# zloyaloha/ray-tracing-practice

Hardware: AMD Instinct MI355X
Metric: Msamples/sec (pixels x spp / s), path-traced frame (higher is better)
Workload: dtype f32

## Files before the change

ray-tracing-practice_amd/csrc/rt_capi.hip:

```cpp
#include <hip/hip_runtime.h>

#include <cmath>
#include <cstdio>
#include <cstdlib>
#include <cstring>
#include <new>
#include <string>
#include <vector>

#include "../../include/rtp_amd.h"
#include "rt_accel.h"
#include "rt_build.h"
#include "rt_device_math.h"
#include "rt_kernel.hip.inc"
#include "rt_primary.hip.inc"
#include "rt_aov.hip.inc"
#include "rt_adaptive.hip.inc"
#include "rt_nee.hip.inc"
#include "rt_env.hip.inc"
#include "rt_light.hip.inc"

namespace {

thread_local std::string g_last_error;
// ... 187 lines not shown
    struct Feedback {
        uint32_t *host = nullptr; hipEvent_t start = nullptr, done = nullptr;
        bool pending = false, guarded = false, exploring = false;
        int passes = 0; uint64_t samples = 0, serial = 0;
    };
    Feedback feedback[kFeedbackSlots];
    int feedback_next = 0;
    double guarded_ns_per_sample = 0.0, exact_ns_per_sample = 0.0;
    bool explore_exact = false;
    uint64_t frame_serial = 0;
    uint32_t trip_test = 0;
    const uint32_t *last_traced_pixels = nullptr;
    int32_t last_spp = 0;
    float4 *leaf_boxes = nullptr, *plane_leaf_boxes = nullptr;
    uint32_t *flag_list = nullptr;
    uint32_t *resume_tag = nullptr; float4 *resume_state = nullptr;
    size_t flag_cap = 0;
    uint32_t *dirty = nullptr, *dirty_list = nullptr;
    size_t dirty_cap = 0;
    hipStream_t aux_stream = nullptr, list_stream = nullptr;
    hipEvent_t ev_fork = nullptr, ev_join = nullptr, ev_listed = nullptr;
    uint32_t *cand = nullptr;
    size_t cand_pixels = 0;
    struct CandKey { float view[12]; int32_t dims[9]; int repacks; hipStream_t stream; bool valid = false; } cand_key;
    int32_t num_internal = 0, num_spheres = 0, num_planes = 0, num_materials = 0, root = rtk::kDone, tree_depth = 0;
    CallClock clock[kNumClocks];
    std::vector<hipEvent_t> pass_events;
    int timed_passes = 0;
    rt_timing last{};
    int last_passes = 0;
    uint64_t last_samples = 0;
    bool timed = false;
    int num_cus = 0;
    uint64_t device_bytes = 0;
    float build_ms = 0.0f;
    bool absorbing_glass = false;
    std::vector<hipEvent_t> aov_events;
    float *adapt_mom = nullptr;
    uint32_t *adapt_list = nullptr, *adapt_work = nullptr, *adapt_counters = nullptr;
    size_t adapt_mom_pixels = 0, adapt_pixels = 0, adapt_work_cap = 0, adapt_counter_words = 0;
    bool nee_built = false;
    std::vector<int32_t> nee_index;
    std::vector<float> nee_cdf, nee_pmf;
    int32_t *nee_index_dev = nullptr;
    float *nee_cdf_dev = nullptr, *nee_pmf_dev = nullptr;
    std::vector<int32_t> emit_code;
    std::vector<float> emit_cdf, emit_pmf, emit_area;
    int32_t emit_spheres = 0, emit_planes = 0;
    int32_t *emit_code_dev = nullptr;
    float *emit_cdf_dev = nullptr, *emit_pmf_dev = nullptr, *emit_area_dev = nullptr;
};

namespace {

template <class T>
rt_status upload(const std::vector<T> &host, void **dev) {
// ... 124 lines not shown
        sc->repack_refused = true;
        return RT_OK;
    }
    HIP_TRY(hipStreamSynchronize(stream));
    float4 *nodes = nullptr, *hnodes = nullptr, *whnodes = nullptr, *leaf_boxes = nullptr, *plane_leaf_boxes = nullptr;
    rt_status st = RT_OK;
    if ((st = upload(pk.nodes, (void **)&nodes)) != RT_OK || (st = upload(pk.hnodes, (void **)&hnodes)) != RT_OK ||
        (st = upload(pk.whnodes, (void **)&whnodes)) != RT_OK ||
        (st = upload(pk.leaf_boxes, (void **)&leaf_boxes)) != RT_OK || (st = upload(pk.plane_leaf_boxes, (void **)&plane_leaf_boxes)) != RT_OK) {
        (void)hipFree(nodes); (void)hipFree(hnodes); (void)hipFree(whnodes); (void)hipFree(leaf_boxes); (void)hipFree(plane_leaf_boxes);
        return st;
    }
    (void)hipFree(sc->nodes); (void)hipFree(sc->hnodes); (void)hipFree(sc->whnodes);
    (void)hipFree(sc->leaf_boxes); (void)hipFree(sc->plane_leaf_boxes);
    sc->nodes = nodes; sc->hnodes = hnodes; sc->whnodes = whnodes; sc->leaf_boxes = leaf_boxes; sc->plane_leaf_boxes = plane_leaf_boxes;
    sc->num_wide = pk.num_wide; sc->wroot = pk.wroot; sc->wide_depth = pk.wide_depth;
    sc->num_internal = pk.num_internal;
    sc->num_top_pairs = pk.num_top_pairs;
    sc->root = pk.root;
    sc->tree_depth = pk.max_depth;
    sc->guard = pk.guard;
    sc->repacks++;
    return RT_OK;
}

}

__attribute__((visibility("hidden"))) void rt_internal_set_error(const std::string &msg) { g_last_error = msg; }

extern "C" {

const char *rt_get_last_error_string(void) { return g_last_error.c_str(); }

#if defined(RTP_PARITY_FLAGS) && !defined(__FAST_MATH__)
#define RTP_VERSION_PARITY "1"
#else
#define RTP_VERSION_PARITY "0"
#endif
#ifdef RTP_DEV_BUILD
#define RTP_VERSION_DEV "1"
#else
#define RTP_VERSION_DEV "0"
#endif
const char *rt_version_string(void) { return "rtp_amd 0.5 gfx950 parity=" RTP_VERSION_PARITY " dev=" RTP_VERSION_DEV; }

rt_status rt_set_device(int32_t device_ordinal) {
// ... 82 lines not shown
    if (cfg.guard_gamma_ulps < 0.0f || !(cfg.guard_gamma_ulps == cfg.guard_gamma_ulps)) return fail(RT_ERR_INVALID_ARG, "guard_gamma_ulps must be >= 0");
    rtaccel::Packed pk;
    const rtaccel::PackOptions popt = pack_options(cfg, desc);
    const bool device_build = cfg.tree_build == RT_BUILD_DEVICE_LBVH;
    std::string err = rtaccel::pack_scene(*desc, device_build ? rtaccel::TreeMode::GuardedLeaves : rtaccel::TreeMode::Guarded, pk, popt);
    if (!err.empty()) return fail(RT_ERR_INVALID_ARG, err);
    if (device_build && !pk.guard.ok) {
        err = rtaccel::pack_scene(*desc, rtaccel::TreeMode::Guarded, pk, popt);
        if (!err.empty()) return fail(RT_ERR_INVALID_ARG, err);
    }

    int n = 0;
    if (hipGetDeviceCount(&n) != hipSuccess || n <= 0) return fail(RT_ERR_NO_DEVICE, "no HIP device");
    rt_scene *sc = new (std::nothrow) rt_scene;
    if (!sc) return fail(RT_ERR_OUT_OF_MEMORY, "host allocation failed");
    sc->cfg = cfg;
    rt_status st = RT_OK;
    auto bail = [&](rt_status s) { rt_scene_destroy(sc); return s; };
    if (hipGetDevice(&sc->device) != hipSuccess) return bail(fail(RT_ERR_HIP, "hipGetDevice failed"));
    hipDeviceProp_t prop;
    if (hipGetDeviceProperties(&prop, sc->device) != hipSuccess) return bail(fail(RT_ERR_HIP, "hipGetDeviceProperties failed"));
    sc->num_cus = prop.multiProcessorCount;
    sc->device_bytes = (uint64_t)prop.totalGlobalMem;
    if (device_build && pk.guard.ok) {
        rtbuild::DeviceTree tree;
        const std::string berr = rtbuild::build_lbvh(pk.guard_leaf_boxes.data(), pk.guard_leaf_codes.data(), (int32_t)pk.guard_leaf_codes.size(), tree);
        if (!berr.empty()) return bail(fail(RT_ERR_HIP, "device BVH build: " + berr));
        sc->nodes = (float4 *)tree.nodes;
        sc->hnodes = (float4 *)tree.hnodes;
        pk.num_internal = tree.num_internal;
        pk.root = tree.root;
        pk.max_depth = tree.depth;
        pk.num_top_pairs = 0;
        sc->build_ms = tree.build_ms;
    } else {
        if ((st = upload(pk.nodes, (void **)&sc->nodes)) != RT_OK) return bail(st);
        if ((st = upload(pk.hnodes, (void **)&sc->hnodes)) != RT_OK) return bail(st);
        if ((st = upload(pk.whnodes, (void **)&sc->whnodes)) != RT_OK) return bail(st);
        sc->num_wide = pk.num_wide; sc->wroot = pk.wroot; sc->wide_depth = pk.wide_depth;
    }
    if ((st = upload(pk.tnodes, (void **)&sc->tnodes)) != RT_OK) return bail(st);
    sc->num_tnodes = pk.num_tnodes;
    if ((st = upload(pk.xnodes, (void **)&sc->xnodes)) != RT_OK) return bail(st);
    sc->num_top = pk.num_top;
    if ((st = upload(pk.spheres, (void **)&sc->spheres)) != RT_OK) return bail(st);
    if ((st = upload(pk.planes, (void **)&sc->planes)) != RT_OK) return bail(st);
// ... 15 lines not shown
        sc->device_built = device_build;
    }
    if (hipMalloc((void **)&sc->queue, kQueueWords * 4) != hipSuccess) return bail(fail(RT_ERR_OUT_OF_MEMORY, "hipMalloc(queue) failed"));
    if (sc->clock[kClockRender].make() != RT_OK) return bail(fail(RT_ERR_HIP, "hipEventCreate failed"));
    sc->num_internal = pk.num_internal;
    sc->num_top_pairs = pk.num_top_pairs;
    sc->num_spheres = (int32_t)pk.sphere_mat.size();
    sc->num_planes = (int32_t)(pk.planes.size() / 20);
    sc->num_materials = (int32_t)(pk.materials.size() / 12);
    sc->root = pk.root;
    sc->tree_depth = pk.max_depth;
    *out_scene = sc;
    return RT_OK;
}

rt_status rt_scene_destroy(rt_scene *sc) {
    if (!sc) return RT_OK;
    (void)hipFree(sc->tnodes);
    (void)hipFree(sc->xnodes);
    (void)hipFree(sc->nodes); (void)hipFree(sc->hnodes); (void)hipFree(sc->whnodes);
    (void)hipFree(sc->spheres); (void)hipFree(sc->planes); (void)hipFree(sc->materials);
    (void)hipFree(sc->sphere_mat); (void)hipFree(sc->tex_data); (void)hipFree(sc->tex_info); (void)hipFree(sc->queue); (void)hipFree(sc->slab);
    (void)hipFree(sc->leaf_boxes); (void)hipFree(sc->plane_leaf_boxes); (void)hipFree(sc->flag_list);
    (void)hipFree(sc->dirty); (void)hipFree(sc->dirty_list); (void)hipFree(sc->cand);
    (void)hipFree(sc->resume_tag); (void)hipFree(sc->resume_state);
    if (sc->aux_stream) (void)hipStreamDestroy(sc->aux_stream);
    if (sc->list_stream) (void)hipStreamDestroy(sc->list_stream);
    if (sc->ev_listed) (void)hipEventDestroy(sc->ev_listed);
    if (sc->ev_fork) (void)hipEventDestroy(sc->ev_fork);
    if (sc->ev_join) (void)hipEventDestroy(sc->ev_join);
    for (hipEvent_t e : sc->pass_events) (void)hipEventDestroy(e);
    for (hipEvent_t e : sc->aov_events) (void)hipEventDestroy(e);
    for (CallClock &c : sc->clock) c.destroy();
    (void)hipFree(sc->adapt_mom); (void)hipFree(sc->adapt_list); (void)hipFree(sc->adapt_work); (void)hipFree(sc->adapt_counters);
    (void)hipFree(sc->nee_index_dev); (void)hipFree(sc->nee_cdf_dev); (void)hipFree(sc->nee_pmf_dev);
    (void)hipFree(sc->emit_code_dev); (void)hipFree(sc->emit_cdf_dev); (void)hipFree(sc->emit_pmf_dev); (void)hipFree(sc->emit_area_dev);
    for (rt_scene::Feedback &f : sc->feedback) {
        if (f.done) { if (f.pending) (void)hipEventSynchronize(f.done); (void)hipEventDestroy(f.done); }
        if (f.start) (void)hipEventDestroy(f.start);
        if (f.host) (void)hipHostFree(f.host);
    }
    delete sc;
    return RT_OK;
}

const char *rt_scene_guard_reason(const rt_scene *sc) {
    if (!sc) return "null scene";
// ... 98 lines not shown
    if (plan.passes < 1) return fail(RT_ERR_UNSUPPORTED, "image too large for the work index arithmetic");
    if (plan.passes > kMaxPasses) return fail(RT_ERR_UNSUPPORTED, "more than 1024 passes (samples_per_pixel above 65536, or above 64512 at 2^24 pixels)");
    int pass_size = plan.pass_size;
    size_t need = (size_t)num_pixels * (size_t)slab_pitch_of(pass_size) * 3;
    if (sc->slab_floats < need) {
        HIP_TRY(hipStreamSynchronize(stream));
        (void)hipFree(sc->slab);
        sc->slab = nullptr;
        sc->slab_floats = 0;
        for (;;) {
            const hipError_t e = hipMalloc((void **)&sc->slab, need * sizeof(float));
            if (e == hipSuccess) break;
            (void)hipGetLastError();
            if (e != hipErrorOutOfMemory || pass_size <= 64) HIP_TRY(e);
            pass_size = pass_size / 2 < 64 ? 64 : pass_size / 2;
            plan = rtaccel::PassPlan::uniform(spp, pass_size);
            need = (size_t)num_pixels * (size_t)slab_pitch_of(pass_size) * 3;
        }
        sc->slab_floats = need;
    }
    return RT_OK;
}
rt_status reserve_view_lists(rt_scene *sc, uint32_t num_pixels, hipStream_t stream, bool &prim) {
    if (!prim || sc->cand_pixels >= (size_t)num_pixels) return RT_OK;
    HIP_TRY(hipStreamSynchronize(stream));
    (void)hipFree(sc->cand);
    sc->cand = nullptr;
    sc->cand_pixels = 0;
    sc->cand_key.valid = false;
    const size_t cand_words = (size_t)num_pixels * (rtk::kCandWords + 1) + 3 * (((size_t)num_pixels + rtk::kOrderBlock - 1) / rtk::kOrderBlock);
    if (hipMalloc((void **)&sc->cand, cand_words * sizeof(uint32_t)) == hipSuccess) {
        sc->cand_pixels = (size_t)num_pixels;
    } else {
        (void)hipGetLastError();
        sc->cand = nullptr;
        prim = false;
    }
    return RT_OK;
}
void bind_view_lists(const rt_scene *sc, rtk::KParams &P, uint32_t num_pixels, bool prim) {
    P.cand = prim ? sc->cand : nullptr;
    P.order = prim ? sc->cand + sc->cand_pixels * rtk::kCandWords : nullptr;
    P.traced_pixels = prim ? P.order + sc->cand_pixels + 2 * (((size_t)num_pixels + rtk::kOrderBlock - 1) / rtk::kOrderBlock) : nullptr;
}
rt_status make_view_lists(rt_scene *sc, const rt_camera_data *cam, const rtk::KParams &P, uint32_t num_pixels, hipStream_t stream) {
    rt_scene::CandKey key{};
    std::memcpy(key.view + 0, cam->origin.e, 12); std::memcpy(key.view + 3, cam->pixel00_loc.e, 12);
    std::memcpy(key.view + 6, cam->pixel_delta_u.e, 12); std::memcpy(key.view + 9, cam->pixel_delta_v.e, 12);
    const int32_t dims[9] = {P.width, P.height, P.local_rows, P.band_rows, P.num_parts, P.part, P.row_w, P.tile_x0, P.tile_y0};
    std::memcpy(key.dims, dims, sizeof(dims));
    key.repacks = sc->repacks; key.stream = stream; key.valid = true;
    const bool cand_cached = sc->cfg.reuse_view_lists >= 0 && sc->cand_key.valid && std::memcmp(key.view, sc->cand_key.view, sizeof(key.view)) == 0 &&
                             std::memcmp(key.dims, sc->cand_key.dims, sizeof(key.dims)) == 0 && key.repacks == sc->cand_key.repacks && key.stream == sc->cand_key.stream;
    if (cand_cached) return RT_OK;
    sc->cand_key.valid = false;
    const double coord_max = rtbeam::coord_bound(cam->origin.e, cam->pixel00_loc.e, cam->pixel_delta_u.e, cam->pixel_delta_v.e, cam->image_width, cam->image_height);
    hipLaunchKernelGGL(rtk::cand_kernel, dim3((num_pixels + 255u) / 256u), dim3(256), 0, stream, P, sc->cand, coord_max);
    HIP_TRY(hipGetLastError());
    uint32_t *order = sc->cand + sc->cand_pixels * rtk::kCandWords, *counts = order + sc->cand_pixels;
    const uint32_t order_blocks = (num_pixels + (uint32_t)rtk::kOrderBlock - 1u) / (uint32_t)rtk::kOrderBlock;
    hipLaunchKernelGGL(rtk::order_count_kernel, dim3(order_blocks), dim3(rtk::kOrderBlock), 0, stream, (const uint32_t *)sc->cand, num_pixels, order_blocks, counts);
    hipLaunchKernelGGL(rtk::order_scan_kernel, dim3(1), dim3(1024), 0, stream, counts, 3u * order_blocks);
    hipLaunchKernelGGL(rtk::order_scatter_kernel, dim3(order_blocks), dim3(rtk::kOrderBlock), 0, stream, (const uint32_t *)sc->cand, num_pixels, order_blocks,
                       (const uint32_t *)counts, order);
    HIP_TRY(hipGetLastError());
    sc->cand_key = key;
    return RT_OK;
}
void launch_primary(const rt_scene *sc, const rtk::KParams &P, uint32_t num_pixels, hipStream_t stream) {
    int pgrid = sc->num_cus * 8;
    const bool by_pixel = P.pass_count >= RTP_BY_PIXEL_MIN;
    const uint32_t units = by_pixel ? (num_pixels + 3u) / 4u : (P.total_work + 255u) / 256u;
    if ((uint32_t)pgrid > units) pgrid = (int)units;
    if (by_pixel) {
        if (P.num_planes > 0) hipLaunchKernelGGL(rtk::primary_pixel_kernel<true>, dim3(pgrid), dim3(256), 0, stream, P);
        else hipLaunchKernelGGL(rtk::primary_pixel_kernel<false>, dim3(pgrid), dim3(256), 0, stream, P);
    } else if (P.num_planes > 0) hipLaunchKernelGGL(rtk::primary_kernel<true>, dim3(pgrid), dim3(256), 0, stream, P);
    else hipLaunchKernelGGL(rtk::primary_kernel<false>, dim3(pgrid), dim3(256), 0, stream, P);
}

bool camera_within(const rt_camera_data *cam, const float c[3], double radius_sq) {
    const double dx = (double)cam->origin.e[0] - c[0], dy = (double)cam->origin.e[1] - c[1], dz = (double)cam->origin.e[2] - c[2];
    return dx * dx + dy * dy + dz * dz <= radius_sq;
}
bool camera_inside_margins(const rt_scene *sc, const rt_camera_data *cam) {
    return camera_within(cam, sc->guard.origin_center, (double)sc->guard.origin_radius * sc->guard.origin_radius) &&
           !(sc->guard.num_small > 0 && !camera_within(cam, sc->guard.center, (double)sc->guard.d0_sq * (1.0 - 1e-5)));
}
bool guarded_chosen(const rt_scene *sc, const rtk::KParams &P) {
    const rt_config &cfg = sc->cfg;
    return sc->guard.ok && cfg.traversal != RT_TRAVERSAL_EXACT && P.root >= 0 && guarded_wanted(cfg, (int64_t)P.num_spheres + P.num_planes) &&
           !(sc->guard_paused && !cfg.guard_keep);
}

rt_status choose_traversal(rt_scene *sc, const rt_camera_data *cam, const rt_shard *shard, const Tile *tile, hipStream_t stream, rtk::KParams &P,
                           bool &guarded, bool &exploring) {
    const rt_config &cfg = sc->cfg;
    guarded = guarded_chosen(sc, P);
    exploring = guarded && sc->explore_exact && cfg.traversal == RT_TRAVERSAL_AUTO && !cfg.guard_keep;
    if (exploring) guarded = false;
    if (!guarded) return RT_OK;
// ... 651 lines not shown
    bind_view_lists(sc, P, num_pixels, prim);
    CallClock &clock = sc->clock[kClockAov];
    if ((st = clock.make(1)) != RT_OK) return st;
    uint32_t *const walked = clock.words;
    const int timed = passes < kTimedPasses ? passes : kTimedPasses;
    if ((st = grow_events(sc->aov_events, 3 * (size_t)timed)) != RT_OK) return st;
    if ((st = clock.start(stream)) != RT_OK) return st;
    HIP_TRY(hipMemsetAsync(walked, 0, sizeof(uint32_t), stream));
    if (prim) {
        if ((st = make_view_lists(sc, cam, P, num_pixels, stream)) != RT_OK) return st;
    } else if (!lens) {
        sc->cand_key.valid = false;
    }
    for (int pass = 0; pass < passes; ++pass) {
        const bool timed_pass = pass < timed;
        if ((st = set_pass(P, plan, pass, num_pixels, sample_first)) != RT_OK) return st;
        if (timed_pass) HIP_TRY(hipEventRecord(sc->aov_events[3 * pass], stream));
        if (prim) {
            launch_primary(sc, P, num_pixels, stream);
            HIP_TRY(hipGetLastError());
        }
        if (timed_pass) HIP_TRY(hipEventRecord(sc->aov_events[3 * pass + 1], stream));
        const uint32_t units = prim ? (num_pixels + 3u) / 4u : (P.total_work + 255u) / 256u;
        const uint32_t rgrid = std::min<uint32_t>(units, (uint32_t)sc->num_cus * 8u);
        if (lens) hipLaunchKernelGGL(rtk::aov_resolve_lens_kernel, dim3(rgrid), dim3(256), 0, stream, P, *lens);
        else if (prim) hipLaunchKernelGGL(rtk::aov_resolve_kernel<false>, dim3(rgrid), dim3(256), 0, stream, P, walked);
        else hipLaunchKernelGGL(rtk::aov_resolve_kernel<true>, dim3(rgrid), dim3(256), 0, stream, P, walked);
        HIP_TRY(hipGetLastError());
        if (timed_pass) HIP_TRY(hipEventRecord(sc->aov_events[3 * pass + 2], stream));
        if (lens) hipLaunchKernelGGL(rtk::aov_accumulate_lens_kernel, acc_grid(num_pixels), dim3(64 * rtk::kAccWaves), 0, stream, P, *lens, out, pass == 0 ? 1 : 0, walked);
        else hipLaunchKernelGGL(rtk::aov_accumulate_kernel, acc_grid(num_pixels), dim3(64 * rtk::kAccWaves), 0, stream, P, out, pass == 0 ? 1 : 0, walked);
        HIP_TRY(hipGetLastError());
    }
    if ((st = clock.stop(stream)) != RT_OK) return st;
    rt_timing t{};
    t.primary_visibility = prim ? 1u : 0u;
    if (sync) {
        if ((st = clock.elapsed(t.kernel_ms)) != RT_OK) return st;
        float primary = 0.0f, rework = 0.0f, ms = 0.0f;
        for (int p = 0; p < timed; ++p) {
            HIP_TRY(hipEventElapsedTime(&ms, sc->aov_events[3 * p], sc->aov_events[3 * p + 1]));
            primary += ms;
            HIP_TRY(hipEventElapsedTime(&ms, sc->aov_events[3 * p + 1], sc->aov_events[3 * p + 2]));
            rework += ms;
        }
        primary *= untimed_scale(passes, timed);
        rework *= untimed_scale(passes, timed);
// ... 68 lines not shown
    if ((st = render_impl(sc, &base, shard, nullptr, d_fb_sum, hip_stream, 0, nullptr, 0, mom)) != RT_OK) return st;
    if (P.max_depth <= 0) {
        HIP_TRY(hipMemsetAsync(mom, 0, (size_t)num_pixels * 8, stream));
        HIP_TRY(hipMemsetD32Async((hipDeviceptr_t)d_spp, a.threshold == 0.0f ? a.min_spp + rounds * batch : a.min_spp, num_pixels, stream));
        if ((st = clock.stop(stream)) != RT_OK) return st;
        if (sync) HIP_TRY(hipStreamSynchronize(stream));
        return RT_OK;
    }
    if (sc->slab_floats < slab_need) return fail(RT_ERR_OUT_OF_MEMORY, "rt_render_adaptive: the sample slab shrank below a round's batch");

    if ((st = fill_params(sc, &base, shard, P)) != RT_OK) return st;
    const LaunchPlan plan = plan_launch(sc, &base, P, false);
    P.fb = d_fb_sum;
    bind_slab(sc, P, num_pixels, batch);
    set_exact_rewalk(P, sc->cfg, plan);
    P.cand = nullptr; P.order = nullptr; P.traced_pixels = nullptr;
    P.resume_tag = nullptr; P.resume_state = nullptr; P.abandon = nullptr; P.dirty = nullptr; P.dirty_list = nullptr;
    P.work_list = sc->adapt_work;
    P.work_cap = num_pixels * (uint32_t)batch;
    const void *exact = rewalk_kernel(plan);
    const int wgs = grid_for(sc, plan.exact, num_pixels, batch);
    const dim3 pix_grid((num_pixels + rtk::kAdaptBlock - 1) / rtk::kAdaptBlock), pix_block(rtk::kAdaptBlock);
    const uint64_t expand_items = (uint64_t)num_pixels * (uint64_t)batch;
    const uint32_t expand_grid = (uint32_t)std::min<uint64_t>((expand_items + rtk::kAdaptBlock - 1) / rtk::kAdaptBlock, (uint64_t)sc->num_cus * 8u);
    uint32_t *lists[2] = {sc->adapt_list, sc->adapt_list + num_pixels};
    uint32_t *const counters = sc->adapt_counters;
    HIP_TRY(hipMemsetAsync(counters, 0, (size_t)3 * (size_t)(rounds + 1) * sizeof(uint32_t), stream));
    int32_t n = a.min_spp;
    hipLaunchKernelGGL(rtk::adaptive_select_kernel<true>, pix_grid, pix_block, 0, stream, (const float *)mom, d_spp, num_pixels, (const uint32_t *)nullptr,
                       (const uint32_t *)nullptr, lists[0], counters, n, batch, a.max_spp, a.threshold);
    HIP_TRY(hipGetLastError());
    for (int32_t r = 1; r <= rounds; ++r) {
        const uint32_t *list = lists[(r - 1) & 1];
        const uint32_t *listed = counters + 3 * (r - 1);
        hipLaunchKernelGGL(rtk::adaptive_expand_kernel, dim3(expand_grid), pix_block, 0, stream, list, listed, (uint32_t)batch, sc->adapt_work,
                           counters + 3 * (r - 1) + 1);
        P.pass_first = n;
        P.pass_count = batch;
        P.total_work = num_pixels * (uint32_t)batch;
        if (!make_magic((uint32_t)batch, (uint64_t)P.total_work + 64, P.magic_count)) return fail(RT_ERR_UNSUPPORTED, "image too large for the work index arithmetic");
        P.work_count = counters + 3 * (r - 1) + 1;
        P.queue = counters + 3 * (r - 1) + 2;
        reservation(P.total_work, (uint64_t)wgs * (rtk::kBlock / rtk::kWave), P.full_chunk, P.full_taper);
        HIP_TRY(launch(exact, (uint32_t)rtk::kBlock, wgs, plan.exact.lds_bytes, stream, P));
        launch_accumulate(stream, P, Acc::onto_sums(list, listed));
        hipLaunchKernelGGL(rtk::moments_kernel<true>, pix_grid, pix_block, 0, stream, mom, (const float *)P.slab, num_pixels, P.slab_pitch, batch, 0, list, listed,
                           (const uint32_t *)nullptr, 0u, 0.0f, 0.0f, 0.0f);
// ... 1074 lines not shown
```

ray-tracing-practice_amd/csrc/rt_kernel.hip.inc:

```
#pragma once

namespace rtk {

using namespace rtd;

constexpr int kWave = 64;
constexpr int32_t kDone = INT32_MIN;
#ifndef RTP_BLOCK
#define RTP_BLOCK 768
#endif
#ifndef RTP_MIN_WAVES
#define RTP_MIN_WAVES 6
#endif
#ifndef RTP_UNROLL
#define RTP_UNROLL 4
#endif
#ifndef RTP_LDS_MAT_ROWS
#define RTP_LDS_MAT_ROWS 1
#endif
#ifndef RTP_UNROLL_WIDE
#define RTP_UNROLL_WIDE 3
#endif
#ifndef RTP_TRIPWIRE
#ifdef RTP_DEV_BUILD
// ... 120 lines not shown

__device__ __forceinline__ f3 inv_exact(const Lane &L) {
    f3 v = L.inv;
    if (__builtin_expect(!(fabsf(v.x) < 1e18f && fabsf(v.y) < 1e18f && fabsf(v.z) < 1e18f), 0)) v = mk(1.0f / L.d.x, 1.0f / L.d.y, 1.0f / L.d.z);
    return v;
}
template <bool kClamped = false>
__device__ __forceinline__ bool slab(const Lane &L0, float lox, float loy, float loz, float hix, float hiy, float hiz,
                                      float t_far, float &t_enter) {
    struct { f3 o, inv; } L = {L0.o, kClamped ? inv_exact(L0) : L0.inv};
    const bool sx = L.inv.x < 0, sy = L.inv.y < 0, sz = L.inv.z < 0;
    const float nx = sx ? hix : lox, fx = sx ? lox : hix;
    const float ny = sy ? hiy : loy, fy = sy ? loy : hiy;
    const float nz = sz ? hiz : loz, fz = sz ? loz : hiz;
    const float t1x = (nx - L.o.x) * L.inv.x, t2x = (fx - L.o.x) * L.inv.x;
    const float t1y = (ny - L.o.y) * L.inv.y, t2y = (fy - L.o.y) * L.inv.y;
    const float t1z = (nz - L.o.z) * L.inv.z, t2z = (fz - L.o.z) * L.inv.z;
    const float tmin = fmaxf(fmaxf(fmaxf(0.001f, t1x), t1y), t1z);
    const float tmax = fminf(fminf(fminf(t_far, t2x), t2y), t2z);
    t_enter = tmin;
    return tmax > tmin;
}

__device__ __forceinline__ bool slab_fused(f3 inv, f3 noi, float lox, float loy, float loz, float hix, float hiy, float hiz,
                                            float t_far, float &t_enter) {
    const float ax = __builtin_fmaf(lox, inv.x, noi.x), bx = __builtin_fmaf(hix, inv.x, noi.x);
    const float ay = __builtin_fmaf(loy, inv.y, noi.y), by = __builtin_fmaf(hiy, inv.y, noi.y);
    const float az = __builtin_fmaf(loz, inv.z, noi.z), bz = __builtin_fmaf(hiz, inv.z, noi.z);
    const float tmin = fmaxf(fmaxf(fminf(ax, bx), fminf(ay, by)), fmaxf(fminf(az, bz), 0.001f));
    const float tmax = fminf(fminf(fmaxf(ax, bx), fmaxf(ay, by)), fminf(fmaxf(az, bz), t_far));
    t_enter = tmin;
    return tmax > tmin;
}

constexpr int32_t kFlagBit = 1 << 30;
constexpr int32_t kEndBit = 1 << 25;
constexpr int32_t kFreshBit = 1 << 24;
constexpr int32_t kArmBit = 1 << 23;
constexpr int32_t kNoResumeBit = 1 << 22;
constexpr int32_t kMaxPrimDepth = 1 << 22;
constexpr int32_t kPrimMiss = -1;
constexpr int32_t kPrimFlag = -2;
constexpr int32_t kPrimWalk = -3;
#ifndef RTP_PRIM_ROUNDS
#define RTP_PRIM_ROUNDS 1
#endif
// ... 273 lines not shown
#endif

template <bool kGuard = false>
__device__ __forceinline__ void test_sphere(Lane &L, float4 s, int32_t prim) {
    const f3 oc = sub(L.o, mk(s.x, s.y, s.z));
    const float a = lensq(L.d);
    const float half_b = dot(oc, L.d);
    const float c = lensq(oc) - s.w * s.w;
    const float disc = half_b * half_b - a * c;
    if (disc < 0) return;
    const double sq = (double)sqrt_cr(disc);
    const double nb = (double)(-half_b);
    const double da = (double)a;
    float t;
    const bool ok = sphere_root(nb, sq, da, L.closest, t);
    if (ok) {
        if (kGuard && t == L.closest && L.hit >= 0) L.depth |= kFlagBit | RTP_WHY(1);
        L.closest = t;
        L.hit = prim;
    }
}

template <bool kGuard = false, bool kLazyFar = false>
__device__ __forceinline__ void test_sphere_ray(Lane &L, float4 s, int32_t prim, float a, double da, double y) {
    const f3 oc = sub(L.o, mk(s.x, s.y, s.z));
    const float half_b = dot(oc, L.d);
    const float c = lensq(oc) - s.w * s.w;
    const float disc = half_b * half_b - a * c;
    if (disc < 0) return;
    const double sq = (double)sqrt_cr(disc);
    const double nb = (double)(-half_b);
    float t;
    if (sphere_root_with<kLazyFar>(nb, sq, da, y, L.closest, t)) {
        if (kGuard && t == L.closest && L.hit >= 0) L.depth |= kFlagBit | RTP_WHY(1);
        L.closest = t;
        L.hit = prim;
    }
}

template <bool kGuard = false, class PlaneTab>
__device__ __forceinline__ void test_plane(Lane &L, PlaneTab planes, int32_t idx, int32_t prim) {
    const float4 P0 = planes[5 * idx + 0];
    const f3 n = mk(P0.x, P0.y, P0.z);
    const float denom = dot(n, L.d);
    if ((double)fabsf(denom) < 1e-8) return;
    const float t = (P0.w - dot(n, L.o)) / denom;
    if (!((0.001f <= t) && (t <= L.closest))) return;
    const float4 P1 = planes[5 * idx + 1];
    const float4 P2 = planes[5 * idx + 2];
    const float4 P3 = planes[5 * idx + 3];
    const float4 P4 = planes[5 * idx + 4];
    const f3 ph = sub(add(L.o, scale(t, L.d)), mk(P4.x, P4.y, P4.z));
    const f3 w = mk(P1.x, P1.y, P1.z);
    const float alpha = dot(w, cross(ph, mk(P3.x, P3.y, P3.z)));
    const float beta = dot(w, cross(mk(P2.x, P2.y, P2.z), ph));
    const int32_t type = as_int(P1.w);
    bool inside = true;
    if (type == RT_PLANE_QUAD) {
        inside = (0.0f <= alpha) && (alpha <= 1.0f) && (0.0f <= beta) && (beta <= 1.0f);
    } else if (type == RT_PLANE_ELLIPSE) {
// ... 869 lines not shown
```

ray-tracing-practice_amd/csrc/rt_primary.hip.inc:

```
#pragma once
#include "rt_beam.h"

namespace rtk {

constexpr int kCandWords = 16;
constexpr uint32_t kCandNone = 0xffffffffu;

__global__ void __launch_bounds__(256) cand_kernel(const KParams P, uint32_t *cand, double coord_max) {
    const uint32_t q = blockIdx.x * 256u + threadIdx.x;
    if (q >= P.num_pixels) return;
    const uint32_t pjl = q / (uint32_t)P.row_w;
    const int32_t pi = (int32_t)(q - pjl * (uint32_t)P.row_w) + P.tile_x0;
    int32_t pj = (int32_t)pjl + P.tile_y0;
    if (P.num_parts != 1) {
        const uint32_t band = pjl / (uint32_t)P.band_rows;
        pj = (int32_t)((band * (uint32_t)P.num_parts + (uint32_t)P.part) * (uint32_t)P.band_rows + (pjl - band * (uint32_t)P.band_rows));
    }
    const rtbeam::Beam beam = rtbeam::make_beam(P.origin, P.p00, P.du, P.dv, pi, pj, coord_max);
    uint32_t codes[kCandWords - 1];
    const float *tab = reinterpret_cast<const float *>(P.nodes);
    int n = rtbeam::beam_candidates(beam, [tab](int32_t k) { return tab + (size_t)k * 16; }, P.root, (double)P.g_dynk, codes, kCandWords - 1);
    n = rtbeam::beam_front_candidates(beam, P.num_front, P.front_code, P.front_box, (double)P.g_dynk, codes, n, kCandWords - 1);
    uint32_t *out = cand + (size_t)q * kCandWords;
    out[0] = n < 0 ? kCandNone : (uint32_t)n;
// ... 1 lines not shown
}

#ifndef RTP_ORDER_SPLIT
#define RTP_ORDER_SPLIT 1
#endif
constexpr int kOrderBlock = 256;
__device__ __forceinline__ uint32_t pixel_class(uint32_t n) { return n == 0u ? 2u : ((RTP_ORDER_SPLIT && n == 1u) ? 1u : 0u); }
__global__ void __launch_bounds__(kOrderBlock) order_count_kernel(const uint32_t *cand, uint32_t num_pixels, uint32_t num_blocks, uint32_t *counts) {
    __shared__ uint32_t part[3][kOrderBlock / 64];
    const uint32_t q = blockIdx.x * (uint32_t)kOrderBlock + threadIdx.x;
    const uint32_t cls = q < num_pixels ? pixel_class(cand[(size_t)q * kCandWords]) : 3u;
    const int wave = threadIdx.x >> 6;
    for (uint32_t c = 0; c < 3; ++c) {
        const uint32_t n = (uint32_t)__popcll(__ballot(cls == c));
        if ((threadIdx.x & 63) == 0) part[c][wave] = n;
    }
    __syncthreads();
    if (threadIdx.x < 3) {
        uint32_t n = 0;
        for (int w = 0; w < kOrderBlock / 64; ++w) n += part[threadIdx.x][w];
        counts[threadIdx.x * num_blocks + blockIdx.x] = n;
    }
}
__global__ void __launch_bounds__(1024) order_scan_kernel(uint32_t *counts, uint32_t n) {
    __shared__ uint32_t sums[1024];
    const uint32_t per = (n + 1023u) / 1024u;
    const uint32_t lo = threadIdx.x * per, hi = lo + per < n ? lo + per : n;
    uint32_t s = 0;
    for (uint32_t k = lo; k < hi; ++k) s += counts[k];
    sums[threadIdx.x] = s;
    __syncthreads();
    for (uint32_t d = 1; d < 1024u; d <<= 1) {
        const uint32_t v = threadIdx.x >= d ? sums[threadIdx.x - d] : 0u;
        __syncthreads();
        sums[threadIdx.x] += v;
        __syncthreads();
    }
    uint32_t run = sums[threadIdx.x] - s;
    for (uint32_t k = lo; k < hi; ++k) { const uint32_t c = counts[k]; counts[k] = run; run += c; }
}
__global__ void __launch_bounds__(kOrderBlock) order_scatter_kernel(const uint32_t *cand, uint32_t num_pixels, uint32_t num_blocks, const uint32_t *offsets,
                                                                    uint32_t *order) {
    __shared__ uint32_t part[3][kOrderBlock / 64];
    const uint32_t q = blockIdx.x * (uint32_t)kOrderBlock + threadIdx.x;
    const uint32_t cls = q < num_pixels ? pixel_class(cand[(size_t)q * kCandWords]) : 3u;
    const int wave = threadIdx.x >> 6;
    uint32_t rank = 0;
    for (uint32_t c = 0; c < 3; ++c) {
// ... 3 lines not shown
    }
    __syncthreads();
    if (cls < 3u) {
        for (int w = 0; w < wave; ++w) rank += part[cls][w];
        order[offsets[cls * num_blocks + blockIdx.x] + rank] = q;
    }
}

typedef __attribute__((address_space(4))) const uint32_t k_u32;
typedef float kf4 __attribute__((ext_vector_type(4)));
typedef __attribute__((address_space(4))) const kf4 k_f4;

struct RayConst { float a; double da, y; };
__device__ __forceinline__ RayConst ray_const(const Lane &L) {
    RayConst r;
    r.a = lensq(L.d);
    r.da = (double)r.a;
    r.y = sphere_root_rcp(r.da);
    return r;
}

typedef uint32_t ku4 __attribute__((ext_vector_type(4)));
typedef __attribute__((address_space(4))) const ku4 k_u4;
template <int C, bool kPlanes>
__device__ __forceinline__ void cand_step(Lane &L, const KParams &P, const RayConst &rc, k_u4 *list4, uint32_t n, k_f4 *sph, ku4 grp, float4 &hs) {
    if constexpr (C < kCandWords - 1) {
        if ((uint32_t)C >= n) return;
        if constexpr ((C + 1) % 4 == 0) grp = list4[(C + 1) / 4];
        const uint32_t code = grp[(C + 1) % 4];
        if (kPlanes && (code & 1u)) {
            test_plane<true>(L, P.planes, (int32_t)(code >> 1), (int32_t)code);
        } else {
            const kf4 sp = sph[code >> 1];
            test_sphere_ray<true, true>(L, make_float4(sp.x, sp.y, sp.z, sp.w), (int32_t)code, rc.a, rc.da, rc.y);
            const bool took = L.hit == (int32_t)code;
            hs = make_float4(took ? sp.x : hs.x, took ? sp.y : hs.y, took ? sp.z : hs.z, took ? sp.w : hs.w);
        }
        cand_step<C + 1, kPlanes>(L, P, rc, list4, n, sph, grp, hs);
    }
}
template <bool kPlanes>
__device__ __forceinline__ int32_t test_uniform_list(Lane &L, const KParams &P, uint32_t q0, float4 &hs) {
    k_u4 *list4 = (k_u4 *)(uintptr_t)(P.cand + (size_t)q0 * kCandWords);
    const ku4 first = list4[0];
    const uint32_t n = first.x;
    if (n == kCandNone) return kPrimWalk;
    const RayConst rc = ray_const(L);
    cand_step<0, kPlanes>(L, P, rc, list4, n, (k_f4 *)(uintptr_t)P.spheres, first, hs);
    return L.hit >= 0 ? L.hit : kPrimMiss;
}
template <bool kPlanes>
__device__ __forceinline__ int32_t test_lane_list(Lane &L, const KParams &P, uint32_t q, float4 &hs) {
    const uint32_t *list = P.cand + (size_t)q * kCandWords;
    const uint32_t n = list[0];
    if (n == kCandNone) return kPrimWalk;
    const RayConst rc = ray_const(L);
    for (uint32_t c = 0; c < n; ++c) {
        const uint32_t code = list[1 + c];
        const int32_t idx = (int32_t)(code >> 1);
        if (kPlanes && (code & 1u)) test_plane<true>(L, P.planes, idx, (int32_t)code);
        else {
            const float4 sp = P.spheres[idx];
            test_sphere_ray<true, true>(L, sp, (int32_t)code, rc.a, rc.da, rc.y);
            if (L.hit == (int32_t)code) hs = sp;
        }
    }
    return L.hit >= 0 ? L.hit : kPrimMiss;
}
template <bool kPlanes>
__device__ __forceinline__ void finish_primary(Lane &L, const KParams &P, int32_t code_out, uint32_t seed1, float4 hs, float *rec) {
    if (P.leaf_boxes == nullptr) {
        float enter;
        const bool in = slab(L, hs.x - hs.w, hs.y - hs.w, hs.z - hs.w, hs.x + hs.w, hs.y + hs.w, hs.z + hs.w, 1e30f, enter);
        const bool sphere_hit = code_out >= 0 && (!kPlanes || !(code_out & 1));
        if (sphere_hit && !(in && L.closest > enter)) L.depth |= kFlagBit;
        if (kPlanes && code_out >= 0 && (code_out & 1) && !guard_final_check<false>(L, P, P.spheres)) L.depth |= kFlagBit;
    } else if (code_out >= 0 && !guard_final_check<false>(L, P, P.spheres)) {
        L.depth |= kFlagBit;
    }
    if (L.depth & kFlagBit) code_out = kPrimFlag;
    rec[0] = L.closest;
    rec[1] = __int_as_float(code_out);
    rec[2] = __uint_as_float(seed1);
}

template <bool kPlanes>
__global__ void __launch_bounds__(256) primary_kernel(const KParams P) {
    const uint32_t lane = threadIdx.x & 63u;
    const uint32_t wave = (blockIdx.x * 256u + threadIdx.x) >> 6, num_waves = gridDim.x * 4u;
    const uint32_t batches = (P.total_work + 63u) >> 6;
    for (uint32_t b = wave; b < batches; b += num_waves) {
        const uint32_t w = b * 64u + lane;
        if (w >= P.total_work) continue;
        int32_t pi, pj;
        uint32_t k, record;
        map_work<false>(P, w, pi, pj, k, 0u, nullptr, nullptr, &record);
        const uint32_t q = P.pass_count == 64 ? (w >> 6) : div_magic(w, P.magic_count);
        if (P.cand[(size_t)q * kCandWords] == 0u) continue;
        Lane L;
        f3 ray_o, ray_d;
        const uint32_t seed1 = sample_seed1(wang_hash((uint32_t)pi * (uint32_t)P.width + (uint32_t)pj), P.pass_first + (int32_t)k);
        camera_ray<false>(L, P, pi, pj, seed1, ray_o, ray_d);
        begin_ray(L, ray_o, ray_d, 0);
        const uint32_t q0 = __builtin_amdgcn_readfirstlane(q);
        float4 hs = make_float4(0.0f, 0.0f, 0.0f, 0.0f);
        const int32_t code_out = __ballot(q != q0) == 0ull ? test_uniform_list<kPlanes>(L, P, q0, hs) : test_lane_list<kPlanes>(L, P, q, hs);
        finish_primary<kPlanes>(L, P, code_out, seed1, hs, P.slab + (size_t)record * 3);
    }
}

template <bool kPlanes>
__global__ void __launch_bounds__(256) primary_pixel_kernel(const KParams P) {
    const uint32_t lane = threadIdx.x & 63u;
    const uint32_t wave = __builtin_amdgcn_readfirstlane((blockIdx.x * 256u + threadIdx.x) >> 6), num_waves = gridDim.x * 4u;
    for (uint32_t q = wave; q < P.num_pixels; q += num_waves) {
        const uint32_t pjl = div_magic(q, P.magic_width);
        const int32_t pi = (int32_t)(q - pjl * (uint32_t)P.row_w) + P.tile_x0;
        int32_t pj = (int32_t)pjl + P.tile_y0;
        if (P.num_parts != 1) {
            const uint32_t band = div_magic(pjl, P.magic_band);
            pj = (int32_t)((band * (uint32_t)P.num_parts + (uint32_t)P.part) * (uint32_t)P.band_rows + (pjl - band * (uint32_t)P.band_rows));
        }
        float *row = P.slab + (size_t)q * P.slab_pitch * 3;
        if (*(k_u32 *)(uintptr_t)(P.cand + (size_t)q * kCandWords) == 0u) continue;
        const uint32_t base_seed = wang_hash((uint32_t)pi * (uint32_t)P.width + (uint32_t)pj);
        for (uint32_t k = lane; k < (uint32_t)P.pass_count; k += 64u) {
            Lane L;
            f3 ray_o, ray_d;
            const uint32_t seed1 = sample_seed1(base_seed, P.pass_first + (int32_t)k);
            camera_ray<false>(L, P, pi, pj, seed1, ray_o, ray_d);
            begin_ray(L, ray_o, ray_d, 0);
            float4 hs = make_float4(0.0f, 0.0f, 0.0f, 0.0f);
            const int32_t code_out = test_uniform_list<kPlanes>(L, P, q, hs);
            finish_primary<kPlanes>(L, P, code_out, seed1, hs, row + (size_t)k * 3);
        }
    }
}

}
```

Measured before the change: 12020.

## Precompute per-sphere camera-relative rows and size grids from occupancy

Adds a per-scene buffer of camera-relative sphere data (origin offset, c term, and box bounds), filled inside the order scan kernel, so primary rays test spheres and their slab boxes without recomputing origin subtraction and radius terms per sample. It adds a fast path for single-candidate pixels. Launch grids for the primary, AOV resolve and adaptive expand kernels are now sized from a measured occupancy query instead of a fixed 8 workgroups per CU. The trade-off is extra memory traffic of three float4 per sphere and possible slight differences in rounding from relative box bounds.

```diff
diff --git a/ray-tracing-practice_amd/csrc/rt_capi.hip b/ray-tracing-practice_amd/csrc/rt_capi.hip
--- a/ray-tracing-practice_amd/csrc/rt_capi.hip
+++ b/ray-tracing-practice_amd/csrc/rt_capi.hip
@@ -233,6 +233,7 @@
     hipEvent_t ev_fork = nullptr, ev_join = nullptr, ev_listed = nullptr;
     uint32_t *cand = nullptr;
     size_t cand_pixels = 0;
+    float4 *view_rows = nullptr;
     struct CandKey { float view[12]; int32_t dims[9]; int repacks; hipStream_t stream; bool valid = false; } cand_key;
     int32_t num_internal = 0, num_spheres = 0, num_planes = 0, num_materials = 0, root = rtk::kDone, tree_depth = 0;
     CallClock clock[kNumClocks];
@@ -243,6 +244,7 @@
     uint64_t last_samples = 0;
     bool timed = false;
     int num_cus = 0;
+    struct Residency { int primary_pixel[2] = {0, 0}, primary[2] = {0, 0}, aov_resolve[2] = {0, 0}, aov_resolve_lens = 0, adapt_expand = 0; } resident;
     uint64_t device_bytes = 0;
     float build_ms = 0.0f;
     bool absorbing_glass = false;
@@ -413,6 +415,34 @@
     sc->guard = pk.guard;
     sc->repacks++;
     return RT_OK;
+}
+
+#ifndef RTP_GRID_WGS_PER_CU
+#define RTP_GRID_WGS_PER_CU 0
+#endif
+rt_status resident_wgs(const void *kernel, int threads, int &out) {
+    int n = 0;
+    HIP_TRY(hipOccupancyMaxActiveBlocksPerMultiprocessor(&n, kernel, threads, 0));
+    if (n < 1) return fail(RT_ERR_HIP, "the occupancy query admits no workgroup of a kernel");
+    const int most = 2048 / threads;
+    out = RTP_GRID_WGS_PER_CU > 0 ? RTP_GRID_WGS_PER_CU : (n < most ? n : most);
+    return RT_OK;
+}
+rt_status measure_residency(rt_scene *sc) {
+    rt_scene::Residency &r = sc->resident;
+    rt_status st;
+    if ((st = resident_wgs(reinterpret_cast<const void *>(&rtk::primary_pixel_kernel<false>), 256, r.primary_pixel[0])) != RT_OK) return st;
+    if ((st = resident_wgs(reinterpret_cast<const void *>(&rtk::primary_pixel_kernel<true>), 256, r.primary_pixel[1])) != RT_OK) return st;
+    if ((st = resident_wgs(reinterpret_cast<const void *>(&rtk::primary_kernel<false>), 256, r.primary[0])) != RT_OK) return st;
+    if ((st = resident_wgs(reinterpret_cast<const void *>(&rtk::primary_kernel<true>), 256, r.primary[1])) != RT_OK) return st;
+    if ((st = resident_wgs(reinterpret_cast<const void *>(&rtk::aov_resolve_kernel<false>), 256, r.aov_resolve[0])) != RT_OK) return st;
+    if ((st = resident_wgs(reinterpret_cast<const void *>(&rtk::aov_resolve_kernel<true>), 256, r.aov_resolve[1])) != RT_OK) return st;
+    if ((st = resident_wgs(reinterpret_cast<const void *>(&rtk::aov_resolve_lens_kernel), 256, r.aov_resolve_lens)) != RT_OK) return st;
+    return resident_wgs(reinterpret_cast<const void *>(&rtk::adaptive_expand_kernel), rtk::kAdaptBlock, r.adapt_expand);
+}
+uint32_t resident_grid(const rt_scene *sc, int wgs_per_cu, uint64_t units) {
+    const uint64_t grid = (uint64_t)sc->num_cus * (uint64_t)wgs_per_cu;
+    return (uint32_t)(units < grid ? units : grid);
 }
 
 }
@@ -541,6 +571,7 @@
     if (hipGetDeviceProperties(&prop, sc->device) != hipSuccess) return bail(fail(RT_ERR_HIP, "hipGetDeviceProperties failed"));
     sc->num_cus = prop.multiProcessorCount;
     sc->device_bytes = (uint64_t)prop.totalGlobalMem;
+    if ((st = measure_residency(sc)) != RT_OK) return bail(st);
     if (device_build && pk.guard.ok) {
         rtbuild::DeviceTree tree;
         const std::string berr = rtbuild::build_lbvh(pk.guard_leaf_boxes.data(), pk.guard_leaf_codes.data(), (int32_t)pk.guard_leaf_codes.size(), tree);
@@ -602,7 +633,7 @@
     (void)hipFree(sc->spheres); (void)hipFree(sc->planes); (void)hipFree(sc->materials);
     (void)hipFree(sc->sphere_mat); (void)hipFree(sc->tex_data); (void)hipFree(sc->tex_info); (void)hipFree(sc->queue); (void)hipFree(sc->slab);
     (void)hipFree(sc->leaf_boxes); (void)hipFree(sc->plane_leaf_boxes); (void)hipFree(sc->flag_list);
-    (void)hipFree(sc->dirty); (void)hipFree(sc->dirty_list); (void)hipFree(sc->cand);
+    (void)hipFree(sc->dirty); (void)hipFree(sc->dirty_list); (void)hipFree(sc->cand); (void)hipFree(sc->view_rows);
     (void)hipFree(sc->resume_tag); (void)hipFree(sc->resume_state);
     if (sc->aux_stream) (void)hipStreamDestroy(sc->aux_stream);
     if (sc->list_stream) (void)hipStreamDestroy(sc->list_stream);
@@ -747,7 +778,15 @@
     return RT_OK;
 }
 rt_status reserve_view_lists(rt_scene *sc, uint32_t num_pixels, hipStream_t stream, bool &prim) {
-    if (!prim || sc->cand_pixels >= (size_t)num_pixels) return RT_OK;
+    if (!prim) return RT_OK;
+    if (sc->view_rows == nullptr && sc->num_spheres > 0 &&
+        hipMalloc((void **)&sc->view_rows, (size_t)sc->num_spheres * rtk::kViewRows * sizeof(float4)) != hipSuccess) {
+        (void)hipGetLastError();
+        sc->view_rows = nullptr;
+        prim = false;
+        return RT_OK;
+    }
+    if (sc->cand_pixels >= (size_t)num_pixels) return RT_OK;
     HIP_TRY(hipStreamSynchronize(stream));
     (void)hipFree(sc->cand);
     sc->cand = nullptr;
@@ -785,7 +824,8 @@
     uint32_t *order = sc->cand + sc->cand_pixels * rtk::kCandWords, *counts = order + sc->cand_pixels;
     const uint32_t order_blocks = (num_pixels + (uint32_t)rtk::kOrderBlock - 1u) / (uint32_t)rtk::kOrderBlock;
     hipLaunchKernelGGL(rtk::order_count_kernel, dim3(order_blocks), dim3(rtk::kOrderBlock), 0, stream, (const uint32_t *)sc->cand, num_pixels, order_blocks, counts);
-    hipLaunchKernelGGL(rtk::order_scan_kernel, dim3(1), dim3(1024), 0, stream, counts, 3u * order_blocks);
+    hipLaunchKernelGGL(rtk::order_scan_kernel, dim3(1), dim3(1024), 0, stream, counts, 3u * order_blocks, (const float4 *)P.spheres, (uint32_t)P.num_spheres, P.origin[0],
+                       P.origin[1], P.origin[2], sc->view_rows);
     hipLaunchKernelGGL(rtk::order_scatter_kernel, dim3(order_blocks), dim3(rtk::kOrderBlock), 0, stream, (const uint32_t *)sc->cand, num_pixels, order_blocks,
                        (const uint32_t *)counts, order);
     HIP_TRY(hipGetLastError());
@@ -793,15 +833,16 @@
     return RT_OK;
 }
 void launch_primary(const rt_scene *sc, const rtk::KParams &P, uint32_t num_pixels, hipStream_t stream) {
-    int pgrid = sc->num_cus * 8;
     const bool by_pixel = P.pass_count >= RTP_BY_PIXEL_MIN;
     const uint32_t units = by_pixel ? (num_pixels + 3u) / 4u : (P.total_work + 255u) / 256u;
-    if ((uint32_t)pgrid > units) pgrid = (int)units;
+    const int planes = P.num_planes > 0 ? 1 : 0;
+    const float4 *rows = sc->view_rows;
+    const uint32_t pgrid = resident_grid(sc, by_pixel ? sc->resident.primary_pixel[planes] : sc->resident.primary[planes], units);
     if (by_pixel) {
-        if (P.num_planes > 0) hipLaunchKernelGGL(rtk::primary_pixel_kernel<true>, dim3(pgrid), dim3(256), 0, stream, P);
-        else hipLaunchKernelGGL(rtk::primary_pixel_kernel<false>, dim3(pgrid), dim3(256), 0, stream, P);
-    } else if (P.num_planes > 0) hipLaunchKernelGGL(rtk::primary_kernel<true>, dim3(pgrid), dim3(256), 0, stream, P);
-    else hipLaunchKernelGGL(rtk::primary_kernel<false>, dim3(pgrid), dim3(256), 0, stream, P);
+        if (planes) hipLaunchKernelGGL(rtk::primary_pixel_kernel<true>, dim3(pgrid), dim3(256), 0, stream, P, rows);
+        else hipLaunchKernelGGL(rtk::primary_pixel_kernel<false>, dim3(pgrid), dim3(256), 0, stream, P, rows);
+    } else if (planes) hipLaunchKernelGGL(rtk::primary_kernel<true>, dim3(pgrid), dim3(256), 0, stream, P, rows);
+    else hipLaunchKernelGGL(rtk::primary_kernel<false>, dim3(pgrid), dim3(256), 0, stream, P, rows);
 }
 
 bool camera_within(const rt_camera_data *cam, const float c[3], double radius_sq) {
@@ -1499,7 +1540,7 @@
         }
         if (timed_pass) HIP_TRY(hipEventRecord(sc->aov_events[3 * pass + 1], stream));
         const uint32_t units = prim ? (num_pixels + 3u) / 4u : (P.total_work + 255u) / 256u;
-        const uint32_t rgrid = std::min<uint32_t>(units, (uint32_t)sc->num_cus * 8u);
+        const uint32_t rgrid = resident_grid(sc, lens ? sc->resident.aov_resolve_lens : sc->resident.aov_resolve[prim ? 0 : 1], units);
         if (lens) hipLaunchKernelGGL(rtk::aov_resolve_lens_kernel, dim3(rgrid), dim3(256), 0, stream, P, *lens);
         else if (prim) hipLaunchKernelGGL(rtk::aov_resolve_kernel<false>, dim3(rgrid), dim3(256), 0, stream, P, walked);
         else hipLaunchKernelGGL(rtk::aov_resolve_kernel<true>, dim3(rgrid), dim3(256), 0, stream, P, walked);
@@ -1614,7 +1655,7 @@
     const int wgs = grid_for(sc, plan.exact, num_pixels, batch);
     const dim3 pix_grid((num_pixels + rtk::kAdaptBlock - 1) / rtk::kAdaptBlock), pix_block(rtk::kAdaptBlock);
     const uint64_t expand_items = (uint64_t)num_pixels * (uint64_t)batch;
-    const uint32_t expand_grid = (uint32_t)std::min<uint64_t>((expand_items + rtk::kAdaptBlock - 1) / rtk::kAdaptBlock, (uint64_t)sc->num_cus * 8u);
+    const uint32_t expand_grid = resident_grid(sc, sc->resident.adapt_expand, (expand_items + rtk::kAdaptBlock - 1) / rtk::kAdaptBlock);
     uint32_t *lists[2] = {sc->adapt_list, sc->adapt_list + num_pixels};
     uint32_t *const counters = sc->adapt_counters;
     HIP_TRY(hipMemsetAsync(counters, 0, (size_t)3 * (size_t)(rounds + 1) * sizeof(uint32_t), stream));
diff --git a/ray-tracing-practice_amd/csrc/rt_kernel.hip.inc b/ray-tracing-practice_amd/csrc/rt_kernel.hip.inc
--- a/ray-tracing-practice_amd/csrc/rt_kernel.hip.inc
+++ b/ray-tracing-practice_amd/csrc/rt_kernel.hip.inc
@@ -166,6 +166,20 @@
     return tmax > tmin;
 }
 
+__device__ __forceinline__ bool slab_rel(f3 inv, f3 lod, f3 hid, float t_far, float &t_enter) {
+    const bool sx = inv.x < 0, sy = inv.y < 0, sz = inv.z < 0;
+    const float ax = lod.x * inv.x, bx = hid.x * inv.x;
+    const float ay = lod.y * inv.y, by = hid.y * inv.y;
+    const float az = lod.z * inv.z, bz = hid.z * inv.z;
+    const float t1x = sx ? bx : ax, t2x = sx ? ax : bx;
+    const float t1y = sy ? by : ay, t2y = sy ? ay : by;
+    const float t1z = sz ? bz : az, t2z = sz ? az : bz;
+    const float tmin = fmaxf(fmaxf(fmaxf(0.001f, t1x), t1y), t1z);
+    const float tmax = fminf(fminf(fminf(t_far, t2x), t2y), t2z);
+    t_enter = tmin;
+    return tmax > tmin;
+}
+
 __device__ __forceinline__ bool slab_fused(f3 inv, f3 noi, float lox, float loy, float loz, float hix, float hiy, float hiz,
                                             float t_far, float &t_enter) {
     const float ax = __builtin_fmaf(lox, inv.x, noi.x), bx = __builtin_fmaf(hix, inv.x, noi.x);
@@ -485,10 +499,8 @@
 }
 
 template <bool kGuard = false, bool kLazyFar = false>
-__device__ __forceinline__ void test_sphere_ray(Lane &L, float4 s, int32_t prim, float a, double da, double y) {
-    const f3 oc = sub(L.o, mk(s.x, s.y, s.z));
+__device__ __forceinline__ void test_sphere_rel(Lane &L, f3 oc, float c, int32_t prim, float a, double da, double y) {
     const float half_b = dot(oc, L.d);
-    const float c = lensq(oc) - s.w * s.w;
     const float disc = half_b * half_b - a * c;
     if (disc < 0) return;
     const double sq = (double)sqrt_cr(disc);
@@ -499,6 +511,11 @@
         L.closest = t;
         L.hit = prim;
     }
+}
+template <bool kGuard = false, bool kLazyFar = false>
+__device__ __forceinline__ void test_sphere_ray(Lane &L, float4 s, int32_t prim, float a, double da, double y) {
+    const f3 oc = sub(L.o, mk(s.x, s.y, s.z));
+    test_sphere_rel<kGuard, kLazyFar>(L, oc, lensq(oc) - s.w * s.w, prim, a, da, y);
 }
 
 template <bool kGuard = false, class PlaneTab>
diff --git a/ray-tracing-practice_amd/csrc/rt_primary.hip.inc b/ray-tracing-practice_amd/csrc/rt_primary.hip.inc
--- a/ray-tracing-practice_amd/csrc/rt_primary.hip.inc
+++ b/ray-tracing-practice_amd/csrc/rt_primary.hip.inc
@@ -47,8 +47,18 @@
         counts[threadIdx.x * num_blocks + blockIdx.x] = n;
     }
 }
-__global__ void __launch_bounds__(1024) order_scan_kernel(uint32_t *counts, uint32_t n) {
+constexpr int kViewRows = 3;
+__device__ __forceinline__ void make_view_rows(float4 s, f3 o, float4 *rows) {
+    const f3 oc = sub(o, mk(s.x, s.y, s.z));
+    const float c = lensq(oc) - s.w * s.w;
+    rows[0] = make_float4(oc.x, oc.y, oc.z, c);
+    rows[1] = make_float4((s.x - s.w) - o.x, (s.y - s.w) - o.y, (s.z - s.w) - o.z, 0.0f);
+    rows[2] = make_float4((s.x + s.w) - o.x, (s.y + s.w) - o.y, (s.z + s.w) - o.z, 0.0f);
+}
+__global__ void __launch_bounds__(1024) order_scan_kernel(uint32_t *counts, uint32_t n, const float4 *spheres, uint32_t num_spheres, float ox, float oy, float oz,
+                                                          float4 *view_rows) {
     __shared__ uint32_t sums[1024];
+    for (uint32_t i = threadIdx.x; i < num_spheres; i += 1024u) make_view_rows(spheres[i], mk(ox, oy, oz), view_rows + (size_t)i * kViewRows);
     const uint32_t per = (n + 1023u) / 1024u;
     const uint32_t lo = threadIdx.x * per, hi = lo + per < n ? lo + per : n;
     uint32_t s = 0;
@@ -98,8 +108,11 @@
 
 typedef uint32_t ku4 __attribute__((ext_vector_type(4)));
 typedef __attribute__((address_space(4))) const ku4 k_u4;
+struct HitBox { f3 lod, hid; };
+__device__ __forceinline__ f3 xyz(kf4 v) { return mk(v.x, v.y, v.z); }
+__device__ __forceinline__ f3 pick(bool took, f3 a, f3 b) { return mk(took ? a.x : b.x, took ? a.y : b.y, took ? a.z : b.z); }
 template <int C, bool kPlanes>
-__device__ __forceinline__ void cand_step(Lane &L, const KParams &P, const RayConst &rc, k_u4 *list4, uint32_t n, k_f4 *sph, ku4 grp, float4 &hs) {
+__device__ __forceinline__ void cand_step(Lane &L, const KParams &P, const RayConst &rc, k_u4 *list4, uint32_t n, k_f4 *rows, ku4 grp, HitBox &hb) {
     if constexpr (C < kCandWords - 1) {
         if ((uint32_t)C >= n) return;
         if constexpr ((C + 1) % 4 == 0) grp = list4[(C + 1) / 4];
@@ -107,47 +120,21 @@
         if (kPlanes && (code & 1u)) {
             test_plane<true>(L, P.planes, (int32_t)(code >> 1), (int32_t)code);
         } else {
-            const kf4 sp = sph[code >> 1];
-            test_sphere_ray<true, true>(L, make_float4(sp.x, sp.y, sp.z, sp.w), (int32_t)code, rc.a, rc.da, rc.y);
+            k_f4 *r = rows + (size_t)(code >> 1) * kViewRows;
+            const kf4 v = r[0], lo = r[1], hi = r[2];
+            test_sphere_rel<true, true>(L, xyz(v), v.w, (int32_t)code, rc.a, rc.da, rc.y);
             const bool took = L.hit == (int32_t)code;
-            hs = make_float4(took ? sp.x : hs.x, took ? sp.y : hs.y, took ? sp.z : hs.z, took ? sp.w : hs.w);
-        }
-        cand_step<C + 1, kPlanes>(L, P, rc, list4, n, sph, grp, hs);
-    }
-}
-template <bool kPlanes>
-__device__ __forceinline__ int32_t test_uniform_list(Lane &L, const KParams &P, uint32_t q0, float4 &hs) {
-    k_u4 *list4 = (k_u4 *)(uintptr_t)(P.cand + (size_t)q0 * kCandWords);
-    const ku4 first = list4[0];
-    const uint32_t n = first.x;
-    if (n == kCandNone) return kPrimWalk;
-    const RayConst rc = ray_const(L);
-    cand_step<0, kPlanes>(L, P, rc, list4, n, (k_f4 *)(uintptr_t)P.spheres, first, hs);
-    return L.hit >= 0 ? L.hit : kPrimMiss;
-}
-template <bool kPlanes>
-__device__ __forceinline__ int32_t test_lane_list(Lane &L, const KParams &P, uint32_t q, float4 &hs) {
-    const uint32_t *list = P.cand + (size_t)q * kCandWords;
-    const uint32_t n = list[0];
-    if (n == kCandNone) return kPrimWalk;
-    const RayConst rc = ray_const(L);
-    for (uint32_t c = 0; c < n; ++c) {
-        const uint32_t code = list[1 + c];
-        const int32_t idx = (int32_t)(code >> 1);
-        if (kPlanes && (code & 1u)) test_plane<true>(L, P.planes, idx, (int32_t)code);
-        else {
-            const float4 sp = P.spheres[idx];
-            test_sphere_ray<true, true>(L, sp, (int32_t)code, rc.a, rc.da, rc.y);
-            if (L.hit == (int32_t)code) hs = sp;
-        }
-    }
-    return L.hit >= 0 ? L.hit : kPrimMiss;
-}
-template <bool kPlanes>
-__device__ __forceinline__ void finish_primary(Lane &L, const KParams &P, int32_t code_out, uint32_t seed1, float4 hs, float *rec) {
+            hb.lod = pick(took, xyz(lo), hb.lod);
+            hb.hid = pick(took, xyz(hi), hb.hid);
+        }
+        cand_step<C + 1, kPlanes>(L, P, rc, list4, n, rows, grp, hb);
+    }
+}
+template <bool kPlanes>
+__device__ __forceinline__ void finish_primary(Lane &L, const KParams &P, int32_t code_out, uint32_t seed1, const HitBox &hb, float *rec) {
     if (P.leaf_boxes == nullptr) {
         float enter;
-        const bool in = slab(L, hs.x - hs.w, hs.y - hs.w, hs.z - hs.w, hs.x + hs.w, hs.y + hs.w, hs.z + hs.w, 1e30f, enter);
+        const bool in = slab_rel(L.inv, hb.lod, hb.hid, 1e30f, enter);
         const bool sphere_hit = code_out >= 0 && (!kPlanes || !(code_out & 1));
         if (sphere_hit && !(in && L.closest > enter)) L.depth |= kFlagBit;
         if (kPlanes && code_out >= 0 && (code_out & 1) && !guard_final_check<false>(L, P, P.spheres)) L.depth |= kFlagBit;
@@ -159,9 +146,58 @@
     rec[1] = __int_as_float(code_out);
     rec[2] = __uint_as_float(seed1);
 }
-
-template <bool kPlanes>
-__global__ void __launch_bounds__(256) primary_kernel(const KParams P) {
+template <bool kPlanes>
+__device__ __forceinline__ void resolve_uniform_list(Lane &L, const KParams &P, k_f4 *rows, uint32_t q0, uint32_t seed1, float *rec) {
+    k_u4 *list4 = (k_u4 *)(uintptr_t)(P.cand + (size_t)q0 * kCandWords);
+    const ku4 first = list4[0];
+    const uint32_t n = first.x;
+    if (n == 1u && !(kPlanes && (first.y & 1u))) {
+        k_f4 *r = rows + (size_t)(first.y >> 1) * kViewRows;
+        const kf4 v = r[0], lo = r[1], hi = r[2];
+        const RayConst rc = ray_const(L);
+        test_sphere_rel<true, true>(L, xyz(v), v.w, (int32_t)first.y, rc.a, rc.da, rc.y);
+        finish_primary<kPlanes>(L, P, L.hit >= 0 ? L.hit : kPrimMiss, seed1, HitBox{xyz(lo), xyz(hi)}, rec);
+        return;
+    }
+    HitBox hb{mk(0.0f, 0.0f, 0.0f), mk(0.0f, 0.0f, 0.0f)};
+    int32_t code_out = kPrimWalk;
+    if (n != kCandNone) {
+        const RayConst rc = ray_const(L);
+        cand_step<0, kPlanes>(L, P, rc, list4, n, rows, first, hb);
+        code_out = L.hit >= 0 ? L.hit : kPrimMiss;
+    }
+    finish_primary<kPlanes>(L, P, code_out, seed1, hb, rec);
+}
+template <bool kPlanes>
+__device__ __forceinline__ void resolve_lane_list(Lane &L, const KParams &P, const float4 *rows, uint32_t q, uint32_t seed1, float *rec) {
+    const uint32_t *list = P.cand + (size_t)q * kCandWords;
+    const uint32_t n = list[0];
+    HitBox hb{mk(0.0f, 0.0f, 0.0f), mk(0.0f, 0.0f, 0.0f)};
+    int32_t code_out = kPrimWalk;
+    if (n != kCandNone) {
+        const RayConst rc = ray_const(L);
+        for (uint32_t c = 0; c < n; ++c) {
+            const uint32_t code = list[1 + c];
+            const int32_t idx = (int32_t)(code >> 1);
+            if (kPlanes && (code & 1u)) test_plane<true>(L, P.planes, idx, (int32_t)code);
+            else {
+                const float4 *r = rows + (size_t)idx * kViewRows;
+                const float4 v = r[0];
+                test_sphere_rel<true, true>(L, mk(v.x, v.y, v.z), v.w, (int32_t)code, rc.a, rc.da, rc.y);
+                if (L.hit == (int32_t)code) {
+                    const float4 lo = r[1], hi = r[2];
+                    hb.lod = mk(lo.x, lo.y, lo.z);
+                    hb.hid = mk(hi.x, hi.y, hi.z);
+                }
+            }
+        }
+        code_out = L.hit >= 0 ? L.hit : kPrimMiss;
+    }
+    finish_primary<kPlanes>(L, P, code_out, seed1, hb, rec);
+}
+
+template <bool kPlanes>
+__global__ void __launch_bounds__(256) primary_kernel(const KParams P, const float4 *view_rows) {
     const uint32_t lane = threadIdx.x & 63u;
     const uint32_t wave = (blockIdx.x * 256u + threadIdx.x) >> 6, num_waves = gridDim.x * 4u;
     const uint32_t batches = (P.total_work + 63u) >> 6;
@@ -179,14 +215,14 @@
         camera_ray<false>(L, P, pi, pj, seed1, ray_o, ray_d);
         begin_ray(L, ray_o, ray_d, 0);
         const uint32_t q0 = __builtin_amdgcn_readfirstlane(q);
-        float4 hs = make_float4(0.0f, 0.0f, 0.0f, 0.0f);
-        const int32_t code_out = __ballot(q != q0) == 0ull ? test_uniform_list<kPlanes>(L, P, q0, hs) : test_lane_list<kPlanes>(L, P, q, hs);
-        finish_primary<kPlanes>(L, P, code_out, seed1, hs, P.slab + (size_t)record * 3);
-    }
-}
-
-template <bool kPlanes>
-__global__ void __launch_bounds__(256) primary_pixel_kernel(const KParams P) {
+        float *rec = P.slab + (size_t)record * 3;
+        if (__ballot(q != q0) == 0ull) resolve_uniform_list<kPlanes>(L, P, (k_f4 *)(uintptr_t)view_rows, q0, seed1, rec);
+        else resolve_lane_list<kPlanes>(L, P, view_rows, q, seed1, rec);
+    }
+}
+
+template <bool kPlanes>
+__global__ void __launch_bounds__(256) primary_pixel_kernel(const KParams P, const float4 *view_rows) {
     const uint32_t lane = threadIdx.x & 63u;
     const uint32_t wave = __builtin_amdgcn_readfirstlane((blockIdx.x * 256u + threadIdx.x) >> 6), num_waves = gridDim.x * 4u;
     for (uint32_t q = wave; q < P.num_pixels; q += num_waves) {
@@ -206,11 +242,9 @@
             const uint32_t seed1 = sample_seed1(base_seed, P.pass_first + (int32_t)k);
             camera_ray<false>(L, P, pi, pj, seed1, ray_o, ray_d);
             begin_ray(L, ray_o, ray_d, 0);
-            float4 hs = make_float4(0.0f, 0.0f, 0.0f, 0.0f);
-            const int32_t code_out = test_uniform_list<kPlanes>(L, P, q, hs);
-            finish_primary<kPlanes>(L, P, code_out, seed1, hs, row + (size_t)k * 3);
-        }
-    }
-}
-
-}
+            resolve_uniform_list<kPlanes>(L, P, (k_f4 *)(uintptr_t)view_rows, q, seed1, row + (size_t)k * 3);
+        }
+    }
+}
+
+}
```

After: 12040, median of 2. No clear change (+0.1%).
